# edouardlp/Mask-RCNN-CoreML

Hardware: AMD Instinct MI355X
Metric: images/sec (1024x1024, COCO-80) (higher is better)
Workload: dtype f32x3

## Files before the change

### mask-rcnn-coreml_amd/csrc/kernels_conv_chain.hip

```cpp
#include "conv_device.h"

namespace mrcnn {

struct ChainArgs { ConvArgs p, q; const void *p_stream, *q_stream; };

__device__ __forceinline__ float4 chain_scale_shift(float4 x, const float4 sc, const float4 sh)
{
    x.x = x.x * sc.x + sh.x; x.y = x.y * sc.y + sh.y; x.z = x.z * sc.z + sh.z; x.w = x.w * sc.w + sh.w;
    return x;
}
__device__ __forceinline__ float4 chain_add(float4 x, const float4 r) { x.x += r.x; x.y += r.y; x.z += r.z; x.w += r.w; return x; }
__device__ __forceinline__ float4 chain_relu(float4 x) { x.x = fmaxf(x.x, 0.f); x.y = fmaxf(x.y, 0.f); x.z = fmaxf(x.z, 0.f); x.w = fmaxf(x.w, 0.f); return x; }
__device__ __forceinline__ bool chain_beyond_fp16(const float4 x) { return !(fabsf(x.x) < 65504.0f) || !(fabsf(x.y) < 65504.0f) || !(fabsf(x.z) < 65504.0f) || !(fabsf(x.w) < 65504.0f); }
__device__ __forceinline__ float4 chain_ld4(const float* p) { return *reinterpret_cast<const float4*>(p); }

struct ChainRows { bool ok[4]; long mrow[4]; int c4; };
__device__ __forceinline__ ChainRows chain_rows(int row0, int M, int lane)
{
    ChainRows rw;
    rw.c4 = (lane & 7) * 4;
#pragma unroll
    for (int ps = 0; ps < 4; ++ps) { const int m = row0 + 8 * ps + (lane >> 3); rw.ok[ps] = m < M; rw.mrow[ps] = m; }
    return rw;
}

struct ChainParts { f16x8 hi, lo, lo2; };
template <int PARTS>
__device__ __forceinline__ ChainParts chain_split(const uint4 u0, const uint4 u1)
{
    ChainParts p;
    if constexpr (PARTS == 3) split_hi_mid_lo(u0, u1, p.hi, p.lo, p.lo2);
    else { split_hi_lo(u0, u1, p.hi, p.lo); p.lo2 = p.lo; }
    return p;
}
template <int PARTS, bool AHEAD, int NG>
__device__ __forceinline__ void chain_split_row(ChainParts (&ap)[NG], const float* in, int row0, int M, int l31, int kk)
{
    const int m = row0 + l31;
    const bool m_ok = m < M;
    const float* const src = in + (long)(m_ok ? m : row0) * (NG * 16) + 8 * kk;
    uint4 u[NG][2];
    if constexpr (AHEAD)
        _Pragma("unroll") for (int g = 0; g < NG; ++g) { u[g][0] = *reinterpret_cast<const uint4*>(src + g * 16); u[g][1] = *reinterpret_cast<const uint4*>(src + g * 16 + 4); }
#pragma unroll
    for (int g = 0; g < NG; ++g) {
        if (!AHEAD || !m_ok) u[g][0] = u[g][1] = make_uint4(0u, 0u, 0u, 0u);
        if (!AHEAD && m_ok) { u[g][0] = *reinterpret_cast<const uint4*>(src + g * 16); u[g][1] = *reinterpret_cast<const uint4*>(src + g * 16 + 4); }
        ap[g] = chain_split<PARTS>(u[g][0], u[g][1]);
    }
}
template <int PARTS, int N, int NA = N, int OFF = 0>
__device__ __forceinline__ void chain_mfma_parts(f32x16 (&acc)[NA], const uint4 (&bv)[N], const ChainParts& pt)
{
    const f16x8 hi = pt.hi, lo = pt.lo, lo2 = pt.lo2;
    _Pragma("unroll") for (int j = 0; j < N; ++j) acc[OFF + j] = __builtin_amdgcn_mfma_f32_32x32x16_f16(__builtin_bit_cast(f16x8, bv[j]), hi, acc[OFF + j], 0, 0, 0);
    _Pragma("unroll") for (int j = 0; j < N; ++j) acc[OFF + j] = __builtin_amdgcn_mfma_f32_32x32x16_f16(__builtin_bit_cast(f16x8, bv[j]), lo, acc[OFF + j], 0, 0, 0);
    if constexpr (PARTS == 3)
        _Pragma("unroll") for (int j = 0; j < N; ++j) acc[OFF + j] = __builtin_amdgcn_mfma_f32_32x32x16_f16(__builtin_bit_cast(f16x8, bv[j]), lo2, acc[OFF + j], 0, 0, 0);
}
template <int N>
__device__ __forceinline__ void chain_zero(f32x16 (&acc)[N])
{
#pragma unroll
    for (int j = 0; j < N; ++j)
#pragma unroll
        for (int e = 0; e < 16; ++e) acc[j][e] = 0.0f;
}

struct ChainTile {
    float* s;
    int lane;
    __device__ __forceinline__ float4* at(int r, int c) const { return reinterpret_cast<float4*>(&s[r * 32 + ((c ^ (r & 7)) << 2)]); }
    __device__ __forceinline__ void put(const f32x16& acc) const
    {
#pragma unroll
        for (int q = 0; q < 4; ++q) *at(lane & 31, 2 * q + (lane >> 5)) = make_float4(acc[4 * q], acc[4 * q + 1], acc[4 * q + 2], acc[4 * q + 3]);
    }
    __device__ __forceinline__ float4 row_get(int ps) const { return *at(8 * ps + (lane >> 3), lane & 7); }
    __device__ __forceinline__ void row_put(int ps, const float4 v) const { *at(8 * ps + (lane >> 3), lane & 7) = v; }
    template <int PARTS>
    __device__ __forceinline__ ChainParts frag(int g) const
    {
        const int c = 4 * g + 2 * (lane >> 5);
        return chain_split<PARTS>(*reinterpret_cast<const uint4*>(at(lane & 31, c)), *reinterpret_cast<const uint4*>(at(lane & 31, c + 1)));
    }
};

__device__ __forceinline__ void chain_residual(float4 (&rv)[2][4], const float* res, const ChainRows& rw, int pitch, int nc)
{
#pragma unroll
    for (int j = 0; j < 2; ++j)
#pragma unroll
        for (int ps = 0; ps < 4; ++ps) {
            rv[j][ps] = make_float4(0.f, 0.f, 0.f, 0.f);
            if (res && rw.ok[ps]) rv[j][ps] = chain_ld4(res + rw.mrow[ps] * pitch + nc + j * 32 + rw.c4);
        }
}
__device__ __forceinline__ void chain_piece_p(const ChainTile& tl, const f32x16& acc, const float* scale, const float* shift, const float4 (&r)[4], bool has_res, bool relu,
                                              const ChainRows& rw, float* out, int pitch, int n, bool& out_of_range)
{
    tl.put(acc);
    __builtin_amdgcn_wave_barrier();
    const float4 sc = chain_ld4(scale + n), sh = chain_ld4(shift + n);
    float4 xs[4];
#pragma unroll
    for (int ps = 0; ps < 4; ++ps) xs[ps] = tl.row_get(ps);
#pragma unroll
    for (int ps = 0; ps < 4; ++ps) {
        float4 x = chain_scale_shift(xs[ps], sc, sh);
        if (has_res) x = chain_add(x, r[ps]);
        if (relu) x = chain_relu(x);
        if (rw.ok[ps]) {
            out_of_range = out_of_range || chain_beyond_fp16(x);
            *reinterpret_cast<float4*>(out + rw.mrow[ps] * pitch + n) = x;
        }
        xs[ps] = x;
    }
    __builtin_amdgcn_wave_barrier();
#pragma unroll
    for (int ps = 0; ps < 4; ++ps) tl.row_put(ps, xs[ps]);
    __builtin_amdgcn_wave_barrier();
}
template <int TNQ>
__device__ __forceinline__ void chain_epilogue_q(const ChainTile& tl, const f32x16 (&acc)[TNQ], const float* scale, const float* shift, bool relu,
                                                 const ChainRows& rw, float* out, bool& out_of_range)
{
#pragma unroll
    for (int jq = 0; jq < TNQ; ++jq) {
        const int n = jq * 32 + rw.c4;
        tl.put(acc[jq]);
        __builtin_amdgcn_wave_barrier();
        const float4 sc = chain_ld4(scale + n), sh = chain_ld4(shift + n);
#pragma unroll
        for (int ps = 0; ps < 4; ++ps) {
            float4 x = chain_scale_shift(tl.row_get(ps), sc, sh);
            if (relu) x = chain_relu(x);
            if (rw.ok[ps]) {
                out_of_range = out_of_range || chain_beyond_fp16(x);
                *reinterpret_cast<float4*>(out + rw.mrow[ps] * (TNQ * 32) + n) = x;
            }
        }
        __builtin_amdgcn_wave_barrier();
    }
}

template <int C, int PARTS, bool SC>
__global__ __launch_bounds__(C == 64 ? 512 : 256, C == 64 ? 1 : 2) void k_conv_chain(const ChainArgs ca)
{
    static_assert(C == 64 || C == 128, "C = 64: filters resident in LDS; C = 128: filters from L2");
    constexpr bool WLDS = C == 64;
    constexpr int NW = WLDS ? 8 : 4, C4 = 4 * C, KT = C / 32, TNP = 2, TNQ = C / 32;
    constexpr int A_BYTES = WLDS ? 0 : KT * 32 * 128;
    constexpr int W_BYTES = WLDS ? C4 * C * 2 : 0;
    constexpr int WF_BYTES = W_BYTES * (SC ? 3 : 2);
    __shared__ __attribute__((aligned(16))) unsigned char smem[WF_BYTES + NW * (A_BYTES + 32 * 32 * 4)];
    const ConvArgs& a = ca.p;
    const ConvArgs& aq = ca.q;
    const int t = threadIdx.x;
    const int wave = t >> 6, lane = t & 63;
    const int l31 = lane & 31, kk = lane >> 5;
    unsigned char* const As = smem + WF_BYTES + wave * A_BYTES;
    const ChainTile tl{reinterpret_cast<float*>(smem + WF_BYTES + NW * A_BYTES) + wave * (32 * 32), lane};
    const float* const in = static_cast<const float*>(a.in);
    const _Float16* const w3 = static_cast<const _Float16*>(a.wgt);
    const _Float16* const w1 = static_cast<const _Float16*>(aq.wgt);
    const float* const res = static_cast<const float*>(a.res);
    float* const out = static_cast<float*>(a.out);
    const _Float16* const wsc = static_cast<const _Float16*>(a.sc_wgt);
    const int swzb = (l31 >> 2) & 3;
    if constexpr (WLDS) {
        auto stage_filter = [&](unsigned char* dst, const _Float16* src, int rows, int K) {
            const int cpr = K / 8;
            for (int idx = t; idx < rows * cpr; idx += NW * 64) {
                const int r = idx / cpr, ch = idx - r * cpr;
                *reinterpret_cast<uint4*>(dst + ((ch >> 2) * rows + r) * 64 + (((ch & 3) ^ ((r >> 2) & 3)) << 4)) = *reinterpret_cast<const uint4*>(src + (long)r * K + ch * 8);
            }
        };
        stage_filter(smem, w3, C4, C);
        stage_filter(smem + W_BYTES, w1, C, C4);
        if constexpr (SC) stage_filter(smem + 2 * W_BYTES, wsc, C4, C);
        __syncthreads();
    }
    bool out_of_range = false, out_of_range_q = false;
    for (int row0 = (blockIdx.x * NW + wave) * 32; row0 < a.M; row0 += gridDim.x * NW * 32) {
    ChainParts ap[WLDS ? 2 * KT : 1];
    if constexpr (WLDS) {
        chain_split_row<PARTS, false>(ap, in, row0, a.M, l31, kk);
    } else {
#pragma unroll
        for (int it = 0; it < C / 8; ++it) {
            const int idx = it * 64 + lane;
            const int r = idx / (C / 4), ch = idx - r * (C / 4);
            const int m = row0 + r;
            uint4 v = make_uint4(0u, 0u, 0u, 0u);
            if (m < a.M) v = *reinterpret_cast<const uint4*>(in + (long)m * C + ch * 4);
            *reinterpret_cast<uint4*>(As + (ch >> 3) * 4096 + r * 128 + (((ch & 7) ^ ((r >> 1) & 7)) << 4)) = v;
        }
        __builtin_amdgcn_wave_barrier();
    }

    const int swz = (l31 >> 1) & 7;
    const unsigned char* const la = As + l31 * 128;
    const int ca0 = ((0 + 2 * kk) ^ swz) << 4, ca1 = ((1 + 2 * kk) ^ swz) << 4, ca2 = ((4 + 2 * kk) ^ swz) << 4, ca3 = ((5 + 2 * kk) ^ swz) << 4;
    const ChainRows rw = chain_rows(row0, a.M, lane);
    const bool relu = a.act == ACT_RELU;

    const float* sc_row = nullptr;
    bool sc_ok = false;
    if constexpr (SC) {
        const int m = row0 + l31;
        sc_ok = m < a.M;
        const int ohw = a.OH * a.OW;
        const int mm = sc_ok ? m : 0;
        const int b = mm / ohw, rem = mm - b * ohw;
        const int oh = rem / a.OW, ow = rem - oh * a.OW;
        sc_row = static_cast<const float*>(a.sc_in) + (long)b * a.sc_in_sB + (long)(oh * a.sc_stride) * a.sc_in_sH + (long)(ow * a.sc_stride) * a.sc_in_sW + 8 * kk;
    }
    uint4 xr[SC && WLDS ? C / 4 : 1];
    if constexpr (SC && WLDS) {
#pragma unroll
        for (int i = 0; i < C / 4; ++i) {
            xr[i] = make_uint4(0u, 0u, 0u, 0u);
            if (sc_ok) xr[i] = *reinterpret_cast<const uint4*>(sc_row + (i >> 1) * 16 + (i & 1) * 4);
        }
    }

    f32x16 accQ[TNQ];
    chain_zero(accQ);
    for (int nc = 0; nc < C4; nc += TNP * 32) {
        float4 rv[TNP][4];
        if constexpr (!SC) chain_residual(rv, res, rw, C4, nc);
        f32x16 accP[TNP], accS[TNP];
        chain_zero(accP);
        chain_zero(accS);
#pragma unroll
        for (int kt = 0; kt < KT; ++kt) {
#pragma unroll
            for (int g = 0; g < 2; ++g) {
                uint4 bv[TNP];
                if constexpr (WLDS) {
#pragma unroll
                    for (int j = 0; j < TNP; ++j) bv[j] = *reinterpret_cast<const uint4*>(smem + (kt * C4 + nc + j * 32 + l31) * 64 + (((2 * g + kk) ^ swzb) << 4));
                    chain_mfma_parts<PARTS, TNP>(accP, bv, ap[2 * kt + g]);
                } else {
                    const uint4 u0 = *reinterpret_cast<const uint4*>(la + kt * 4096 + (g ? ca2 : ca0));
                    const uint4 u1 = *reinterpret_cast<const uint4*>(la + kt * 4096 + (g ? ca3 : ca1));
#pragma unroll
                    for (int j = 0; j < TNP; ++j) bv[j] = *reinterpret_cast<const uint4*>(w3 + (long)(nc + j * 32 + l31) * C + kt * 32 + g * 16 + 8 * kk);
                    chain_mfma_parts<PARTS, TNP>(accP, bv, chain_split<PARTS>(u0, u1));
                }
            }
        }
        if constexpr (SC) {
            for (int g = 0; g < (WLDS ? C / 16 : a.sc_Cin / 16); ++g) {
                uint4 u0 = make_uint4(0u, 0u, 0u, 0u), u1 = u0;
                if constexpr (WLDS) { u0 = xr[2 * g]; u1 = xr[2 * g + 1]; }
                else if (sc_ok) { u0 = *reinterpret_cast<const uint4*>(sc_row + g * 16); u1 = *reinterpret_cast<const uint4*>(sc_row + g * 16 + 4); }
                uint4 bv[TNP];
#pragma unroll
                for (int j = 0; j < TNP; ++j) {
                    if constexpr (WLDS) bv[j] = *reinterpret_cast<const uint4*>(smem + 2 * W_BYTES + ((g >> 1) * C4 + nc + j * 32 + l31) * 64 + (((2 * (g & 1) + kk) ^ swzb) << 4));
                    else bv[j] = *reinterpret_cast<const uint4*>(wsc + (long)(nc + j * 32 + l31) * a.sc_Cin + g * 16 + 8 * kk);
                }
                chain_mfma_parts<PARTS, TNP>(accS, bv, chain_split<PARTS>(u0, u1));
            }
        }
#pragma unroll
        for (int j = 0; j < TNP; ++j) {
            const int n = nc + j * 32 + rw.c4;
            if constexpr (SC) {
                tl.put(accS[j]);
                __builtin_amdgcn_wave_barrier();
                const float4 sc2 = chain_ld4(a.sc_scale + n), sh2 = chain_ld4(a.sc_shift + n);
#pragma unroll
                for (int ps = 0; ps < 4; ++ps) {
                    rv[j][ps] = chain_scale_shift(tl.row_get(ps), sc2, sh2);
                    out_of_range = out_of_range || chain_beyond_fp16(rv[j][ps]);
                }
                __builtin_amdgcn_wave_barrier();
            }
            tl.put(accP[j]);
            __builtin_amdgcn_wave_barrier();
            const float4 sc = chain_ld4(a.scale + n), sh = chain_ld4(a.shift + n);
            float4 xs[4];
#pragma unroll
            for (int ps = 0; ps < 4; ++ps) {
                float4 x = chain_scale_shift(tl.row_get(ps), sc, sh);
                if (SC || res) x = chain_add(x, rv[j][ps]);
                if (relu) x = chain_relu(x);
                if (rw.ok[ps]) {
                    out_of_range = out_of_range || chain_beyond_fp16(x);
                    *reinterpret_cast<float4*>(out + rw.mrow[ps] * C4 + n) = x;
                }
                xs[ps] = x;
            }
            __builtin_amdgcn_wave_barrier();
#pragma unroll
            for (int ps = 0; ps < 4; ++ps) tl.row_put(ps, xs[ps]);
            __builtin_amdgcn_wave_barrier();
#pragma unroll
            for (int g = 0; g < 2; ++g) {
                uint4 bq[TNQ];
#pragma unroll
                for (int jq = 0; jq < TNQ; ++jq) {
                    if constexpr (WLDS) bq[jq] = *reinterpret_cast<const uint4*>(smem + W_BYTES + ((nc / 32 + j) * C + jq * 32 + l31) * 64 + (((2 * g + kk) ^ swzb) << 4));
                    else bq[jq] = *reinterpret_cast<const uint4*>(w1 + (long)(jq * 32 + l31) * C4 + nc + j * 32 + g * 16 + 8 * kk);
                }
                chain_mfma_parts<PARTS, TNQ>(accQ, bq, tl.template frag<PARTS>(g));
            }
            __builtin_amdgcn_wave_barrier();
        }
    }
    chain_epilogue_q(tl, accQ, aq.scale, aq.shift, aq.act == ACT_RELU, rw, static_cast<float*>(aq.out), out_of_range_q);
    }
    if (a.range_flag && out_of_range) atomicOr(a.range_flag, 1);
    if (aq.range_flag && out_of_range_q) atomicOr(aq.range_flag, 1);
}

template <int C, int PARTS>
__global__ __launch_bounds__(256, 1) void k_conv_chain_ring(const ChainArgs ca)
{
    static_assert(C == 256, "the ring's stage holds C = 256's chunk images");
    constexpr int C4 = 4 * C, KT = C / 32, TNP = 2, TNQ = C / 32, NCH = C4 / 64;
    constexpr int WCH = 64 * C * 2;
    constexpr int STAGE = 2 * WCH;
    constexpr int NDMA = WCH / 4096;
    __shared__ __attribute__((aligned(16))) unsigned char smem[2 * STAGE + 4 * 32 * 32 * 4];
    __shared__ __attribute__((aligned(16))) float s_tab[2 * C4], s_tabq[2 * C];
    const ConvArgs& a = ca.p;
    const ConvArgs& aq = ca.q;
    const int t = threadIdx.x;
    const int wave = t >> 6, lane = t & 63;
    const int l31 = lane & 31, kk = lane >> 5;
    const ChainTile tl{reinterpret_cast<float*>(smem + 2 * STAGE) + wave * (32 * 32), lane};
    static_assert(C4 == 4 * 256 && C % 8 == 0 && C / 2 <= 256, "the tables are filled by 256 threads, 16 B each");
    *reinterpret_cast<float4*>(&s_tab[4 * t]) = chain_ld4(a.scale + 4 * t);
    *reinterpret_cast<float4*>(&s_tab[C4 + 4 * t]) = chain_ld4(a.shift + 4 * t);
    if (t < C / 2) *reinterpret_cast<float4*>(&s_tabq[4 * t]) = chain_ld4(t < C / 4 ? aq.scale + 4 * t : aq.shift + 4 * (t - C / 4));
    const float* const res = static_cast<const float*>(a.res);
    float* const out = static_cast<float*>(a.out);
    const int swzb = (l31 >> 2) & 3;

    typedef unsigned srd_t __attribute__((ext_vector_type(4)));
    srd_t srdP, srdQ;
    {
        const unsigned long long wp = (unsigned long long)(uintptr_t)ca.p_stream, wq = (unsigned long long)(uintptr_t)ca.q_stream;
        srdP[0] = __builtin_amdgcn_readfirstlane((unsigned)wp);
        srdP[1] = __builtin_amdgcn_readfirstlane((unsigned)(wp >> 32) & 0xffffu);
        srdP[2] = (unsigned)(NCH * WCH);
        srdP[3] = 0x00020000u;
        srdQ[0] = __builtin_amdgcn_readfirstlane((unsigned)wq);
        srdQ[1] = __builtin_amdgcn_readfirstlane((unsigned)(wq >> 32) & 0xffffu);
        srdQ[2] = (unsigned)(NCH * WCH);
        srdQ[3] = 0x00020000u;
    }
    const unsigned lds0 = __builtin_amdgcn_readfirstlane((unsigned)(uintptr_t)(__attribute__((address_space(3))) unsigned char*)smem);
    const unsigned wdst = lds0 + (unsigned)__builtin_amdgcn_readfirstlane(wave) * 1024u;
    const unsigned voff = (unsigned)t * 16u;
#define MRCNN_RING_DMA(SRD, SOFF, DST)                                                                         \
    asm volatile("s_nop 4\n\ts_mov_b32 m0, %3\n\ts_nop 0\n\tbuffer_load_dwordx4 %0, %1, %2 offen lds" ::"v"(voff), "s"(SRD), "s"(SOFF), "s"(DST) : "memory", "m0");
    auto ring_fill = [&](int ch) {
        const unsigned src = (unsigned)__builtin_amdgcn_readfirstlane(ch) * (unsigned)WCH;
        const unsigned dst = wdst + (unsigned)(__builtin_amdgcn_readfirstlane(ch) & 1) * (unsigned)STAGE;
#pragma unroll
        for (int k = 0; k < NDMA; ++k) {
            MRCNN_RING_DMA(srdP, src + k * 4096u, dst + k * 4096u)
            MRCNN_RING_DMA(srdQ, src + k * 4096u, dst + (unsigned)WCH + k * 4096u)
        }
    };
    ring_fill(0);

    const int row0 = (blockIdx.x * 4 + __builtin_amdgcn_readfirstlane(wave)) * 32;
    const bool live = row0 < a.M;
    bool out_of_range = false, out_of_range_q = false;
    ChainParts ap[2 * KT];
    if (live) chain_split_row<PARTS, true>(ap, static_cast<const float*>(a.in), row0, a.M, l31, kk);
    const bool full = row0 + 32 <= a.M;
    const ChainRows rw = chain_rows(row0, a.M, lane);
    const bool relu = a.act == ACT_RELU;
    f32x16 accQ[TNQ];
    chain_zero(accQ);

    for (int ch = 0; ch < NCH; ++ch) {
        if (full) asm volatile("s_waitcnt vmcnt(4)" ::: "memory");
        else asm volatile("s_waitcnt vmcnt(0)" ::: "memory");
        __syncthreads();
        if (ch + 1 < NCH) ring_fill(ch + 1);
        if (!live) continue;
        const unsigned char* const w3s = smem + (ch & 1) * STAGE;
        const unsigned char* const w1s = w3s + WCH;
        const int nc = ch * 64;
        float4 rv[TNP][4];
        chain_residual(rv, res, rw, C4, nc);
        f32x16 accP[TNP];
        chain_zero(accP);
        auto frag_p = [&](uint4 (&b)[TNP], int i) {
#pragma unroll
            for (int j = 0; j < TNP; ++j) b[j] = *reinterpret_cast<const uint4*>(w3s + ((i >> 1) * 64 + j * 32 + l31) * 64 + (((2 * (i & 1) + kk) ^ swzb) << 4));
        };
        {
            uint4 bv[TNP];
            frag_p(bv, 0);
#pragma unroll
            for (int i = 0; i < 2 * KT; ++i) {
                uint4 bn[TNP];
                if (i + 1 < 2 * KT) frag_p(bn, i + 1);
                __builtin_amdgcn_sched_barrier(0);
                chain_mfma_parts<PARTS, TNP>(accP, bv, ap[i]);
                if (i + 1 < 2 * KT) {
#pragma unroll
                    for (int j = 0; j < TNP; ++j) bv[j] = bn[j];
                }
            }
        }
        auto frag_q = [&](uint4 (&b)[TNQ / 2], int j, int h) {
#pragma unroll
            for (int i = 0; i < TNQ / 2; ++i) b[i] = *reinterpret_cast<const uint4*>(w1s + (j * C + ((h & 1) * (TNQ / 2) + i) * 32 + l31) * 64 + (((2 * (h >> 1) + kk) ^ swzb) << 4));
        };
#pragma unroll
        for (int j = 0; j < TNP; ++j) {
            const int n = nc + j * 32 + rw.c4;
            uint4 bq[TNQ / 2];
            frag_q(bq, j, 0);
            chain_piece_p(tl, accP[j], s_tab, s_tab + C4, rv[j], res != nullptr, relu, rw, out, C4, n, out_of_range);
            ChainParts pt;
#pragma unroll
            for (int h = 0; h < 4; ++h) {
                if ((h & 1) == 0) pt = tl.template frag<PARTS>(h >> 1);
                uint4 bn[TNQ / 2];
                if (h < 3) frag_q(bn, j, h + 1);
                __builtin_amdgcn_sched_barrier(0);
                if (h & 1) chain_mfma_parts<PARTS, TNQ / 2, TNQ, TNQ / 2>(accQ, bq, pt);
                else chain_mfma_parts<PARTS, TNQ / 2, TNQ, 0>(accQ, bq, pt);
                if (h < 3) {
#pragma unroll
                    for (int i = 0; i < TNQ / 2; ++i) bq[i] = bn[i];
                }
            }
            __builtin_amdgcn_wave_barrier();
        }
    }
#undef MRCNN_RING_DMA
    if (live) chain_epilogue_q(tl, accQ, s_tabq, s_tabq + C, aq.act == ACT_RELU, rw, static_cast<float*>(aq.out), out_of_range_q);
    if (a.range_flag && out_of_range) atomicOr(a.range_flag, 1);
    if (aq.range_flag && out_of_range_q) atomicOr(aq.range_flag, 1);
}

typedef void (*chain_kernel_t)(const ChainArgs);
template <int PARTS>
static chain_kernel_t chain_kernel(int C, bool sc)
{
    if (C == 256) return k_conv_chain_ring<256, PARTS>;
    if (C == 64) return sc ? k_conv_chain<64, PARTS, true> : k_conv_chain<64, PARTS, false>;
    return sc ? k_conv_chain<128, PARTS, true> : k_conv_chain<128, PARTS, false>;
}

void conv_chain_launch(hipStream_t s, const ConvArgs& p, const ConvArgs& q, int parts, int n_cus, const void* p_stream, const void* q_stream)
{
    ChainArgs ca{p, q, p_stream, q_stream};
    dim3 grid((p.M + 127) / 128), block(256);
    const bool sc = p.sc_in != nullptr;
    const int C = q.Cout;
    MRCNN_REQUIRE((C == 64 || C == 128 || C == 256) && (parts == 2 || parts == 3), MRCNN_ERR_INVALID, "conv_chain_launch: C %d, %d parts", C, parts);
    if (C == 256) MRCNN_REQUIRE(!sc && p.res && p_stream && q_stream, MRCNN_ERR_INVALID, "conv_chain_launch: C = 256 runs identity pairs from their stream images");
    if (C == 64) {
        MRCNN_REQUIRE((!sc || p.sc_Cin == 64) && n_cus > 0, MRCNN_ERR_INVALID, "conv_chain_launch: the LDS-resident form holds C = 64's filters");
        const int tiles256 = (p.M + 255) / 256;
        grid = dim3(tiles256 < n_cus ? tiles256 : n_cus); block = dim3(512);
    }
    hipLaunchKernelGGL(parts == 3 ? chain_kernel<3>(C, sc) : chain_kernel<2>(C, sc), grid, block, 0, s, ca);
}

}
```

Baseline: 455.8.

## Split C=256 conv chain ring into producer and consumer wave pairs

The C=256 chained conv kernel now runs 512 threads. Four waves compute the first (expand) conv's MFMA tiles and drive the weight DMA ring. The other four waves consume finished 32-column pieces through per-pair LDS tiles, applying the scale/shift/residual epilogue and accumulating the second conv. Weight staging is split into half-chunks, and the second conv's filters get their own three-slot ring, so both convs' MFMA work and the DMA overlap across waves instead of running serially in one wave. The epilogue is specialized on full-tile and relu, with precomputed byte offsets. The price is more barrier synchronisation, larger LDS use, and a fragile block-wide __syncthreads count that must match between the two roles.

```diff
diff --git a/mask-rcnn-coreml_amd/csrc/kernels_conv_chain.hip b/mask-rcnn-coreml_amd/csrc/kernels_conv_chain.hip
--- a/mask-rcnn-coreml_amd/csrc/kernels_conv_chain.hip
+++ b/mask-rcnn-coreml_amd/csrc/kernels_conv_chain.hip
@@ -33,19 +33,17 @@
     else { split_hi_lo(u0, u1, p.hi, p.lo); p.lo2 = p.lo; }
     return p;
 }
-template <int PARTS, bool AHEAD, int NG>
+template <int PARTS, int NG>
 __device__ __forceinline__ void chain_split_row(ChainParts (&ap)[NG], const float* in, int row0, int M, int l31, int kk)
 {
     const int m = row0 + l31;
     const bool m_ok = m < M;
     const float* const src = in + (long)(m_ok ? m : row0) * (NG * 16) + 8 * kk;
     uint4 u[NG][2];
-    if constexpr (AHEAD)
-        _Pragma("unroll") for (int g = 0; g < NG; ++g) { u[g][0] = *reinterpret_cast<const uint4*>(src + g * 16); u[g][1] = *reinterpret_cast<const uint4*>(src + g * 16 + 4); }
 #pragma unroll
     for (int g = 0; g < NG; ++g) {
-        if (!AHEAD || !m_ok) u[g][0] = u[g][1] = make_uint4(0u, 0u, 0u, 0u);
-        if (!AHEAD && m_ok) { u[g][0] = *reinterpret_cast<const uint4*>(src + g * 16); u[g][1] = *reinterpret_cast<const uint4*>(src + g * 16 + 4); }
+        u[g][0] = u[g][1] = make_uint4(0u, 0u, 0u, 0u);
+        if (m_ok) { u[g][0] = *reinterpret_cast<const uint4*>(src + g * 16); u[g][1] = *reinterpret_cast<const uint4*>(src + g * 16 + 4); }
         ap[g] = chain_split<PARTS>(u[g][0], u[g][1]);
     }
 }
@@ -96,27 +94,41 @@
             if (res && rw.ok[ps]) rv[j][ps] = chain_ld4(res + rw.mrow[ps] * pitch + nc + j * 32 + rw.c4);
         }
 }
-__device__ __forceinline__ void chain_piece_p(const ChainTile& tl, const f32x16& acc, const float* scale, const float* shift, const float4 (&r)[4], bool has_res, bool relu,
-                                              const ChainRows& rw, float* out, int pitch, int n, bool& out_of_range)
-{
-    tl.put(acc);
-    __builtin_amdgcn_wave_barrier();
+struct ChainRowOffs { bool ok[4]; unsigned off[4]; };
+__device__ __forceinline__ ChainRowOffs chain_row_offs(int row0, int M, int lane, int pitch)
+{
+    ChainRowOffs ro;
+#pragma unroll
+    for (int ps = 0; ps < 4; ++ps) {
+        const int r = 8 * ps + (lane >> 3);
+        ro.ok[ps] = row0 + r < M;
+        ro.off[ps] = (unsigned)((ro.ok[ps] ? r : 0) * pitch + (lane & 7) * 4) * 4u;
+    }
+    return ro;
+}
+__device__ __forceinline__ void chain_residual_piece(float4 (&rv)[4], const float* res, const ChainRowOffs& ro)
+{
+#pragma unroll
+    for (int ps = 0; ps < 4; ++ps) rv[ps] = *reinterpret_cast<const float4*>(reinterpret_cast<const char*>(res) + ro.off[ps]);
+}
+template <bool FULL, bool RELU>
+__device__ __forceinline__ void chain_piece_p(const ChainTile& tl, const float* scale, const float* shift, const float4 (&r)[4], const ChainRowOffs& ro, float* out, int n,
+                                              bool& out_of_range)
+{
     const float4 sc = chain_ld4(scale + n), sh = chain_ld4(shift + n);
     float4 xs[4];
 #pragma unroll
     for (int ps = 0; ps < 4; ++ps) xs[ps] = tl.row_get(ps);
 #pragma unroll
     for (int ps = 0; ps < 4; ++ps) {
-        float4 x = chain_scale_shift(xs[ps], sc, sh);
-        if (has_res) x = chain_add(x, r[ps]);
-        if (relu) x = chain_relu(x);
-        if (rw.ok[ps]) {
-            out_of_range = out_of_range || chain_beyond_fp16(x);
-            *reinterpret_cast<float4*>(out + rw.mrow[ps] * pitch + n) = x;
+        float4 x = chain_add(chain_scale_shift(xs[ps], sc, sh), r[ps]);
+        if (RELU) x = chain_relu(x);
+        if (FULL || ro.ok[ps]) {
+            out_of_range |= chain_beyond_fp16(x);
+            *reinterpret_cast<float4*>(reinterpret_cast<char*>(out) + ro.off[ps]) = x;
         }
         xs[ps] = x;
     }
-    __builtin_amdgcn_wave_barrier();
 #pragma unroll
     for (int ps = 0; ps < 4; ++ps) tl.row_put(ps, xs[ps]);
     __builtin_amdgcn_wave_barrier();
@@ -185,7 +197,7 @@
     for (int row0 = (blockIdx.x * NW + wave) * 32; row0 < a.M; row0 += gridDim.x * NW * 32) {
     ChainParts ap[WLDS ? 2 * KT : 1];
     if constexpr (WLDS) {
-        chain_split_row<PARTS, false>(ap, in, row0, a.M, l31, kk);
+        chain_split_row<PARTS>(ap, in, row0, a.M, l31, kk);
     } else {
 #pragma unroll
         for (int it = 0; it < C / 8; ++it) {
@@ -318,133 +330,194 @@
 }
 
 template <int C, int PARTS>
-__global__ __launch_bounds__(256, 1) void k_conv_chain_ring(const ChainArgs ca)
-{
-    static_assert(C == 256, "the ring's stage holds C = 256's chunk images");
-    constexpr int C4 = 4 * C, KT = C / 32, TNP = 2, TNQ = C / 32, NCH = C4 / 64;
+__global__ __launch_bounds__(512, 1) void k_conv_chain_ring(const ChainArgs ca)
+{
+    static_assert(C == 256, "the ring's stages hold C = 256's chunk images");
+    constexpr int C4 = 4 * C, KT = C / 32, TNP = 2, TNQ = C / 32, NCH = C4 / 64, NPC = 2 * NCH;
     constexpr int WCH = 64 * C * 2;
-    constexpr int STAGE = 2 * WCH;
-    constexpr int NDMA = WCH / 4096;
-    __shared__ __attribute__((aligned(16))) unsigned char smem[2 * STAGE + 4 * 32 * 32 * 4];
+    constexpr int WHALF = WCH / 2;
+    constexpr int NW1 = 3;
+    constexpr int W1_OFF = 2 * WCH, TILE_OFF = W1_OFF + NW1 * WHALF;
+    __shared__ __attribute__((aligned(16))) unsigned char smem[TILE_OFF + 4 * 2 * 32 * 32 * 4];
     __shared__ __attribute__((aligned(16))) float s_tab[2 * C4], s_tabq[2 * C];
     const ConvArgs& a = ca.p;
     const ConvArgs& aq = ca.q;
-    const int t = threadIdx.x;
-    const int wave = t >> 6, lane = t & 63;
+    const int wave = __builtin_amdgcn_readfirstlane((int)threadIdx.x >> 6), lane = threadIdx.x & 63;
+    const int pair = wave & 3;
     const int l31 = lane & 31, kk = lane >> 5;
-    const ChainTile tl{reinterpret_cast<float*>(smem + 2 * STAGE) + wave * (32 * 32), lane};
-    static_assert(C4 == 4 * 256 && C % 8 == 0 && C / 2 <= 256, "the tables are filled by 256 threads, 16 B each");
-    *reinterpret_cast<float4*>(&s_tab[4 * t]) = chain_ld4(a.scale + 4 * t);
-    *reinterpret_cast<float4*>(&s_tab[C4 + 4 * t]) = chain_ld4(a.shift + 4 * t);
-    if (t < C / 2) *reinterpret_cast<float4*>(&s_tabq[4 * t]) = chain_ld4(t < C / 4 ? aq.scale + 4 * t : aq.shift + 4 * (t - C / 4));
+    float* const tiles = reinterpret_cast<float*>(smem + TILE_OFF) + pair * (2 * 32 * 32);
+    const ChainTile tx{tiles, lane}, ty{tiles + 32 * 32, lane};
+    const int swzb = (l31 >> 2) & 3;
+    const int row0 = (blockIdx.x * 4 + pair) * 32;
+    const bool live = row0 < a.M;
+
+    if (wave < 4) {
+        const int t = pair * 64 + lane;
+        static_assert(C4 == 4 * 256 && C % 8 == 0 && C / 2 <= 256, "the tables are filled by 256 threads, 16 B each");
+        *reinterpret_cast<float4*>(&s_tab[4 * t]) = chain_ld4(a.scale + 4 * t);
+        *reinterpret_cast<float4*>(&s_tab[C4 + 4 * t]) = chain_ld4(a.shift + 4 * t);
+        if (t < C / 2) *reinterpret_cast<float4*>(&s_tabq[4 * t]) = chain_ld4(t < C / 4 ? aq.scale + 4 * t : aq.shift + 4 * (t - C / 4));
+        typedef unsigned srd_t __attribute__((ext_vector_type(4)));
+        srd_t srdP, srdQ;
+        {
+            const unsigned long long wp = (unsigned long long)(uintptr_t)ca.p_stream, wq = (unsigned long long)(uintptr_t)ca.q_stream;
+            srdP[0] = __builtin_amdgcn_readfirstlane((unsigned)wp);
+            srdP[1] = __builtin_amdgcn_readfirstlane((unsigned)(wp >> 32) & 0xffffu);
+            srdP[2] = (unsigned)(NCH * WCH);
+            srdP[3] = 0x00020000u;
+            srdQ[0] = __builtin_amdgcn_readfirstlane((unsigned)wq);
+            srdQ[1] = __builtin_amdgcn_readfirstlane((unsigned)(wq >> 32) & 0xffffu);
+            srdQ[2] = (unsigned)(NCH * WCH);
+            srdQ[3] = 0x00020000u;
+        }
+        const unsigned lds0 = __builtin_amdgcn_readfirstlane((unsigned)(uintptr_t)(__attribute__((address_space(3))) unsigned char*)smem);
+        const unsigned wdst = lds0 + (unsigned)pair * 1024u;
+        const unsigned voff = (unsigned)t * 16u;
+#define MRCNN_RING_DMA(SRD, SOFF, DST)                                                                         \
+    asm volatile("s_nop 4\n\ts_mov_b32 m0, %3\n\ts_nop 0\n\tbuffer_load_dwordx4 %0, %1, %2 offen lds" ::"v"(voff), "s"(SRD), "s"(SOFF), "s"(DST) : "memory", "m0");
+        auto fill_w3 = [&](int c, int h) {
+            const unsigned src = (unsigned)__builtin_amdgcn_readfirstlane(c) * (unsigned)WCH + (unsigned)(h * WHALF);
+            const unsigned dst = wdst + (unsigned)(__builtin_amdgcn_readfirstlane(c) & 1) * (unsigned)WCH + (unsigned)(h * WHALF);
+#pragma unroll
+            for (int k = 0; k < WHALF / 4096; ++k) MRCNN_RING_DMA(srdP, src + k * 4096u, dst + k * 4096u)
+        };
+        auto fill_w1 = [&](int p) {
+            const unsigned off = (unsigned)(__builtin_amdgcn_readfirstlane(p) & 1) * (unsigned)WHALF;
+            const unsigned src = (unsigned)(__builtin_amdgcn_readfirstlane(p) >> 1) * (unsigned)WCH + off;
+            const unsigned dst = wdst + (unsigned)W1_OFF + ((unsigned)__builtin_amdgcn_readfirstlane(p) % (unsigned)NW1) * (unsigned)WHALF;
+#pragma unroll
+            for (int k = 0; k < WHALF / 4096; ++k) MRCNN_RING_DMA(srdQ, src + k * 4096u, dst + k * 4096u)
+        };
+        fill_w3(0, 0);
+        fill_w3(0, 1);
+        auto ring_step = [&](int c, int h) {
+            if (c + 1 < NCH) fill_w3(c + 1, h);
+            fill_w1(2 * c + h);
+        };
+        uint4 u[2 * KT][2];
+        {
+            const int m = row0 + l31;
+            const float* const src = static_cast<const float*>(a.in) + (long)m * C + 8 * kk;
+#pragma unroll
+            for (int g = 0; g < 2 * KT; ++g) {
+                u[g][0] = u[g][1] = make_uint4(0u, 0u, 0u, 0u);
+                if (m < a.M) { u[g][0] = *reinterpret_cast<const uint4*>(src + g * 16); u[g][1] = *reinterpret_cast<const uint4*>(src + g * 16 + 4); }
+            }
+        }
+        f32x16 accP[TNP];
+        chain_zero(accP);
+        for (int c = 0; c < NCH; ++c) {
+            const unsigned char* const w3s = smem + (c & 1) * WCH;
+            auto frag_p = [&](uint4 (&b)[TNP], int i) {
+#pragma unroll
+                for (int j = 0; j < TNP; ++j) b[j] = *reinterpret_cast<const uint4*>(w3s + ((i >> 1) * 64 + j * 32 + l31) * 64 + (((2 * (i & 1) + kk) ^ swzb) << 4));
+            };
+#pragma unroll
+            for (int h = 0; h < 2; ++h) {
+                if (2 * c + h == 0 || c + 1 >= NCH) asm volatile("s_waitcnt vmcnt(0)" ::: "memory");
+                else asm volatile("s_waitcnt vmcnt(8)" ::: "memory");
+                __syncthreads();
+                if (!live) { ring_step(c, h); continue; }
+                if (h == 0) {
+                    if (c > 0) ty.put(accP[1]);
+                    chain_zero(accP);
+                }
+                uint4 bv[TNP];
+                frag_p(bv, 8 * h);
+                ChainParts pt = chain_split<PARTS>(u[8 * h][0], u[8 * h][1]);
+#pragma unroll
+                for (int i = 8 * h; i < 8 * h + 8; ++i) {
+                    uint4 bn[TNP];
+                    ChainParts pn;
+                    if (i + 1 < 8 * h + 8) { frag_p(bn, i + 1); pn = chain_split<PARTS>(u[i + 1][0], u[i + 1][1]); }
+                    chain_mfma_parts<PARTS, TNP>(accP, bv, pt);
+                    if (i + 1 < 8 * h + 8) {
+#pragma unroll
+                        for (int j = 0; j < TNP; ++j) bv[j] = bn[j];
+                        pt = pn;
+                    }
+                }
+                ring_step(c, h);
+                if (h == 1) tx.put(accP[0]);
+            }
+        }
+        asm volatile("s_waitcnt vmcnt(0)" ::: "memory");
+        __syncthreads();
+        if (live) ty.put(accP[1]);
+        asm volatile("s_waitcnt vmcnt(0)" ::: "memory");
+        __syncthreads();
+#undef MRCNN_RING_DMA
+        return;
+    }
+
+    if (!live) {
+        for (int s = 0; s < NPC + 2; ++s) __syncthreads();
+        return;
+    }
     const float* const res = static_cast<const float*>(a.res);
     float* const out = static_cast<float*>(a.out);
-    const int swzb = (l31 >> 2) & 3;
-
-    typedef unsigned srd_t __attribute__((ext_vector_type(4)));
-    srd_t srdP, srdQ;
-    {
-        const unsigned long long wp = (unsigned long long)(uintptr_t)ca.p_stream, wq = (unsigned long long)(uintptr_t)ca.q_stream;
-        srdP[0] = __builtin_amdgcn_readfirstlane((unsigned)wp);
-        srdP[1] = __builtin_amdgcn_readfirstlane((unsigned)(wp >> 32) & 0xffffu);
-        srdP[2] = (unsigned)(NCH * WCH);
-        srdP[3] = 0x00020000u;
-        srdQ[0] = __builtin_amdgcn_readfirstlane((unsigned)wq);
-        srdQ[1] = __builtin_amdgcn_readfirstlane((unsigned)(wq >> 32) & 0xffffu);
-        srdQ[2] = (unsigned)(NCH * WCH);
-        srdQ[3] = 0x00020000u;
-    }
-    const unsigned lds0 = __builtin_amdgcn_readfirstlane((unsigned)(uintptr_t)(__attribute__((address_space(3))) unsigned char*)smem);
-    const unsigned wdst = lds0 + (unsigned)__builtin_amdgcn_readfirstlane(wave) * 1024u;
-    const unsigned voff = (unsigned)t * 16u;
-#define MRCNN_RING_DMA(SRD, SOFF, DST)                                                                         \
-    asm volatile("s_nop 4\n\ts_mov_b32 m0, %3\n\ts_nop 0\n\tbuffer_load_dwordx4 %0, %1, %2 offen lds" ::"v"(voff), "s"(SRD), "s"(SOFF), "s"(DST) : "memory", "m0");
-    auto ring_fill = [&](int ch) {
-        const unsigned src = (unsigned)__builtin_amdgcn_readfirstlane(ch) * (unsigned)WCH;
-        const unsigned dst = wdst + (unsigned)(__builtin_amdgcn_readfirstlane(ch) & 1) * (unsigned)STAGE;
-#pragma unroll
-        for (int k = 0; k < NDMA; ++k) {
-            MRCNN_RING_DMA(srdP, src + k * 4096u, dst + k * 4096u)
-            MRCNN_RING_DMA(srdQ, src + k * 4096u, dst + (unsigned)WCH + k * 4096u)
-        }
-    };
-    ring_fill(0);
-
-    const int row0 = (blockIdx.x * 4 + __builtin_amdgcn_readfirstlane(wave)) * 32;
-    const bool live = row0 < a.M;
+    const bool full = row0 + 32 <= a.M;
+    const ChainRowOffs ro = chain_row_offs(row0, a.M, lane, C4);
+    const float* const res0 = res + (long)row0 * C4;
+    float* const out0 = out + (long)row0 * C4;
+    const int c4 = (lane & 7) * 4;
+    const bool relu = a.act == ACT_RELU;
     bool out_of_range = false, out_of_range_q = false;
-    ChainParts ap[2 * KT];
-    if (live) chain_split_row<PARTS, true>(ap, static_cast<const float*>(a.in), row0, a.M, l31, kk);
-    const bool full = row0 + 32 <= a.M;
-    const ChainRows rw = chain_rows(row0, a.M, lane);
-    const bool relu = a.act == ACT_RELU;
     f32x16 accQ[TNQ];
     chain_zero(accQ);
-
-    for (int ch = 0; ch < NCH; ++ch) {
-        if (full) asm volatile("s_waitcnt vmcnt(4)" ::: "memory");
-        else asm volatile("s_waitcnt vmcnt(0)" ::: "memory");
-        __syncthreads();
-        if (ch + 1 < NCH) ring_fill(ch + 1);
-        if (!live) continue;
-        const unsigned char* const w3s = smem + (ch & 1) * STAGE;
-        const unsigned char* const w1s = w3s + WCH;
-        const int nc = ch * 64;
-        float4 rv[TNP][4];
-        chain_residual(rv, res, rw, C4, nc);
-        f32x16 accP[TNP];
-        chain_zero(accP);
-        auto frag_p = [&](uint4 (&b)[TNP], int i) {
-#pragma unroll
-            for (int j = 0; j < TNP; ++j) b[j] = *reinterpret_cast<const uint4*>(w3s + ((i >> 1) * 64 + j * 32 + l31) * 64 + (((2 * (i & 1) + kk) ^ swzb) << 4));
-        };
-        {
-            uint4 bv[TNP];
-            frag_p(bv, 0);
-#pragma unroll
-            for (int i = 0; i < 2 * KT; ++i) {
-                uint4 bn[TNP];
-                if (i + 1 < 2 * KT) frag_p(bn, i + 1);
+    float4 rv[2][4];
+    auto residual = [&](float4 (&r)[4], int p) { chain_residual_piece(r, res0 + p * 32, ro); };
+    residual(rv[0], 0);
+    __syncthreads();
+    __syncthreads();
+    for (int c = 0; c < NCH; ++c) {
+#pragma unroll
+        for (int j = 0; j < 2; ++j) {
+            const int p = 2 * c + j;
+            residual(rv[j ^ 1], p + 1 < NPC ? p + 1 : p);
+            __syncthreads();
+            const ChainTile& tl = j ? ty : tx;
+            const unsigned char* const w1s = smem + W1_OFF + ((unsigned)p % (unsigned)NW1) * WHALF;
+            auto frag_q = [&](uint4 (&b)[TNQ / 4], int h) {
+#pragma unroll
+                for (int i = 0; i < TNQ / 4; ++i) b[i] = *reinterpret_cast<const uint4*>(w1s + (((h & 3) * (TNQ / 4) + i) * 32 + l31) * 64 + (((2 * (h >> 2) + kk) ^ swzb) << 4));
+            };
+            uint4 bq[TNQ / 4];
+            frag_q(bq, 0);
+            const int n = p * 32 + c4;
+            if (full) {
+                if (relu) chain_piece_p<true, true>(tl, s_tab, s_tab + C4, rv[j], ro, out0 + p * 32, n, out_of_range);
+                else chain_piece_p<true, false>(tl, s_tab, s_tab + C4, rv[j], ro, out0 + p * 32, n, out_of_range);
+            } else {
+                if (relu) chain_piece_p<false, true>(tl, s_tab, s_tab + C4, rv[j], ro, out0 + p * 32, n, out_of_range);
+                else chain_piece_p<false, false>(tl, s_tab, s_tab + C4, rv[j], ro, out0 + p * 32, n, out_of_range);
+            }
+            ChainParts pt;
+#pragma unroll
+            for (int h = 0; h < 8; ++h) {
+                if ((h & 3) == 0) pt = tl.template frag<PARTS>(h >> 2);
+                uint4 bn[TNQ / 4];
+                if (h < 7) frag_q(bn, h + 1);
                 __builtin_amdgcn_sched_barrier(0);
-                chain_mfma_parts<PARTS, TNP>(accP, bv, ap[i]);
-                if (i + 1 < 2 * KT) {
-#pragma unroll
-                    for (int j = 0; j < TNP; ++j) bv[j] = bn[j];
-                }
-            }
-        }
-        auto frag_q = [&](uint4 (&b)[TNQ / 2], int j, int h) {
-#pragma unroll
-            for (int i = 0; i < TNQ / 2; ++i) b[i] = *reinterpret_cast<const uint4*>(w1s + (j * C + ((h & 1) * (TNQ / 2) + i) * 32 + l31) * 64 + (((2 * (h >> 1) + kk) ^ swzb) << 4));
-        };
-#pragma unroll
-        for (int j = 0; j < TNP; ++j) {
-            const int n = nc + j * 32 + rw.c4;
-            uint4 bq[TNQ / 2];
-            frag_q(bq, j, 0);
-            chain_piece_p(tl, accP[j], s_tab, s_tab + C4, rv[j], res != nullptr, relu, rw, out, C4, n, out_of_range);
-            ChainParts pt;
-#pragma unroll
-            for (int h = 0; h < 4; ++h) {
-                if ((h & 1) == 0) pt = tl.template frag<PARTS>(h >> 1);
-                uint4 bn[TNQ / 2];
-                if (h < 3) frag_q(bn, j, h + 1);
-                __builtin_amdgcn_sched_barrier(0);
-                if (h & 1) chain_mfma_parts<PARTS, TNQ / 2, TNQ, TNQ / 2>(accQ, bq, pt);
-                else chain_mfma_parts<PARTS, TNQ / 2, TNQ, 0>(accQ, bq, pt);
-                if (h < 3) {
-#pragma unroll
-                    for (int i = 0; i < TNQ / 2; ++i) bq[i] = bn[i];
+                if ((h & 3) == 0) chain_mfma_parts<PARTS, TNQ / 4, TNQ, 0>(accQ, bq, pt);
+                else if ((h & 3) == 1) chain_mfma_parts<PARTS, TNQ / 4, TNQ, TNQ / 4>(accQ, bq, pt);
+                else if ((h & 3) == 2) chain_mfma_parts<PARTS, TNQ / 4, TNQ, TNQ / 2>(accQ, bq, pt);
+                else chain_mfma_parts<PARTS, TNQ / 4, TNQ, 3 * TNQ / 4>(accQ, bq, pt);
+                if (h < 7) {
+#pragma unroll
+                    for (int i = 0; i < TNQ / 4; ++i) bq[i] = bn[i];
                 }
             }
             __builtin_amdgcn_wave_barrier();
         }
     }
-#undef MRCNN_RING_DMA
-    if (live) chain_epilogue_q(tl, accQ, s_tabq, s_tabq + C, aq.act == ACT_RELU, rw, static_cast<float*>(aq.out), out_of_range_q);
+    int lane_q = lane;
+    asm volatile("" : "+v"(lane_q));
+    chain_epilogue_q(tx, accQ, s_tabq, s_tabq + C, aq.act == ACT_RELU, chain_rows(row0, a.M, lane_q), static_cast<float*>(aq.out), out_of_range_q);
     if (a.range_flag && out_of_range) atomicOr(a.range_flag, 1);
     if (aq.range_flag && out_of_range_q) atomicOr(aq.range_flag, 1);
 }
+
 
 typedef void (*chain_kernel_t)(const ChainArgs);
 template <int PARTS>
@@ -458,9 +531,9 @@
 void conv_chain_launch(hipStream_t s, const ConvArgs& p, const ConvArgs& q, int parts, int n_cus, const void* p_stream, const void* q_stream)
 {
     ChainArgs ca{p, q, p_stream, q_stream};
-    dim3 grid((p.M + 127) / 128), block(256);
     const bool sc = p.sc_in != nullptr;
     const int C = q.Cout;
+    dim3 grid((p.M + 127) / 128), block(C == 256 ? 512 : 256);
     MRCNN_REQUIRE((C == 64 || C == 128 || C == 256) && (parts == 2 || parts == 3), MRCNN_ERR_INVALID, "conv_chain_launch: C %d, %d parts", C, parts);
     if (C == 256) MRCNN_REQUIRE(!sc && p.res && p_stream && q_stream, MRCNN_ERR_INVALID, "conv_chain_launch: C = 256 runs identity pairs from their stream images");
     if (C == 64) {
```

After: 465.9, median of 6. 2.2% higher.
